# GlaireDaggers/Pretty-Fast-Video

Measured on AMD Instinct MI355X. Metric: macroblocks/s (encode+decode) 1080p YUV420, higher is better.
Workload: dtype i32 (encoder transforms evaluated in exact f32; decoders i32)

## Files before the change

pretty-fast-video_amd/csrc/pfv_kernels.hip:

```cpp
#include <hip/hip_runtime.h>
#include <stdint.h>

#include "pfv_device.h"
#include "pfv_prof.h"


namespace pfv {

namespace {
__constant__ int kScale[64] = {
    32, 37, 34, 26, 32, 26, 34, 37, 37, 43, 39, 31, 37, 31, 39, 43, 34, 39, 35, 28, 34, 28, 35, 39, 26, 31, 28, 22, 26, 22,
    28, 31, 32, 37, 34, 26, 32, 26, 34, 37, 26, 31, 28, 22, 26, 22, 28, 31, 34, 39, 35, 28, 34, 28, 35, 39, 37, 43, 39, 31,
    37, 31, 39, 43,
};
__constant__ int kInvZigzag[64] = {
    0,  1,  5,  6,  14, 15, 27, 28, 2,  4,  7,  13, 16, 26, 29, 42, 3,  8,  12, 17, 25, 30, 41, 43, 9,  11, 18, 24, 31, 40,
    44, 53, 10, 19, 23, 32, 39, 45, 52, 54, 20, 22, 33, 38, 46, 51, 55, 60, 21, 34, 37, 47, 50, 56, 59, 61, 35, 36, 48, 49,
    57, 58, 62, 63,
};
}

constexpr int kWinRows = 16 * kStripsPerWG + 30;
constexpr int kWinStride = 176;
constexpr int kWinBytes = kWinRows * kWinStride;
// ... 512 lines not shown
{
    return quant_div(quant_scale(m, scale16), rcp, magic, biased);
}
__device__ __forceinline__ f2 residual_f(f2 src, f2 pred)
{
    const f2 d = src - pred;
    const float c = 0.5f - 1.0f / 2048.0f;
    const f2 r = f2{__builtin_fmaf(d[0], c, kQuantMagic), __builtin_fmaf(d[1], c, kQuantMagic)};
    return f2{__builtin_fmaf(r[0], 256.0f, -256.0f * kQuantMagic), __builtin_fmaf(r[1], 256.0f, -256.0f * kQuantMagic)};
}
__device__ __forceinline__ int16_t quant_low16(float biased) { return (int16_t)__float_as_int(biased); }
__device__ __forceinline__ void forward_half_f(f2 (&x)[8], int *xw, int m, int i, const LaneQ &lq, float magic)
{
    int *mb = xw + m * kMBPitch;
    ffdct8(x);
    f_rows_to_cols(x, mb, i, m & 3);
    ffdct8(x);
    int16_t *stage = reinterpret_cast<int16_t *>(xw) + m * (2 * kStagePitch);
#pragma unroll
    for (int k = 0; k < 8; k++) {
        const int zz = lq.zz(k);
        f2 biased;
        x[k] = quant_pair_f(x[k], lq.scale(k), lq.rcp(k), magic, biased);
#pragma unroll
        for (int s = 0; s < 2; s++) stage[s * 64 + zz] = quant_low16(biased[s]);
    }
    wave_lds_sync();
}
constexpr float kPixelBias = 127.501953125f;
__device__ __forceinline__ f2 iframe_pixel_f(f2 x) { return x * f2s(1.0f / 256.0f) + f2s(kPixelBias); }
template <bool PIXEL>
__device__ __forceinline__ void inverse_half_f(f2 (&c)[8], int *xw, int m, int i, const LaneQ &lq)
{
    int *mb = xw + m * kMBPitch;
#pragma unroll
    for (int k = 0; k < 8; k++) c[k] = c[k] * f2s(lq.deqf(k));
    fidct8(c);
    f_cols_to_rows(c, mb, i, m & 3);
    fidct8(c);
#pragma unroll
    for (int k = 0; k < 8; k++) c[k] = PIXEL ? iframe_pixel_f(c[k]) : f2floor(c[k] * f2s(1.0f / 256.0f));
}
__device__ __forceinline__ uint4 pack_row_f(const f2 (&px)[8])
{
    unsigned w[4] = {0, 0, 0, 0};
#pragma unroll
    for (int k = 0; k < 8; k++) {
        w[k >> 2] = __builtin_amdgcn_cvt_pk_u8_f32(px[k][0], (unsigned)(k & 3), w[k >> 2]);
        w[2 + (k >> 2)] = __builtin_amdgcn_cvt_pk_u8_f32(px[k][1], (unsigned)(k & 3), w[2 + (k >> 2)]);
    }
    return make_uint4(w[0], w[1], w[2], w[3]);
}
__device__ __forceinline__ void unpack_row_f(const uint4 &row, f2 (&px)[8])
{
#pragma unroll
    for (int k = 0; k < 4; k++) {
        px[k] = f2{(float)byte_of(row.x, k), (float)byte_of(row.z, k)};
        px[k + 4] = f2{(float)byte_of(row.y, k), (float)byte_of(row.w, k)};
    }
}

template <bool FLT, int LPM = 8>
__global__ __launch_bounds__(kThreads) void k_enc_iframe(FrameGeom g, const uint8_t *__restrict__ src,
                                                          int16_t *__restrict__ coef, uint8_t *__restrict__ recon,
                                                          const QTab *__restrict__ qtabs, float qmagic)
{
    __shared__ __attribute__((aligned(16))) int xchg[kStripsPerWG][kXchgDwords];
    __shared__ __attribute__((aligned(16))) int qtab_lds[kStripsPerWG][kQTabDwords];
    constexpr int kPasses = LPM == 8 ? 2 : 1;

    const int lane = threadIdx.x & 63, wave = __builtin_amdgcn_readfirstlane((int)(threadIdx.x >> 6));
    const int gw = xcd_remap((int)blockIdx.x, (int)gridDim.x) * kStripsPerWG + wave;
    const int gstrip = LPM == 8 ? gw : gw >> 1, half_strip = LPM == 8 ? 0 : gw & 1;
    if (gstrip >= g.strips_per_frame * g.n_streams) return;
    const StripPos sp = locate_strip(g, gstrip);
    if (half_strip * 4 >= sp.n_mb) return;
    const PlaneGeom &p = g.p[sp.plane];
    const int slot = lane >> 3, i = lane & 7;
    const int m = LPM == 8 ? slot : half_strip * 4 + (slot >> 1);
    int *xw = xchg[wave];

    fill_qtable<true, FLT>(qtab_lds[wave], qtabs + p.qsel, lane);
    const uint8_t *plane = frame_src(g, src, sp.stream) + p.src_off;
    uint4 rows[kPasses];
#pragma unroll
    for (int pass = 0; pass < kPasses; pass++) rows[pass] = load_src16(plane, p, sp.x0 + m * 16, sp.y0 + i + 8 * (LPM == 8 ? pass : (slot & 1)));

    wave_lds_sync();
    const LaneQ lq{qtab_lds[wave], i};
    int16_t *coef_mb0 = coef + ((long)sp.stream * g.mbs_per_frame + sp.mb_first) * 256;
    uint8_t *dst = recon ? recon + (long)sp.stream * g.pad_frame_bytes + p.pad_off + (long)(sp.y0 + i) * p.pw + sp.x0 + m * 16
                         : nullptr;
#pragma unroll
    for (int pass = 0; pass < kPasses; pass++) {
        const int h = LPM == 8 ? pass : (slot & 1);
        if (FLT) {
            f2 x[8];
            unpack_row_f(rows[pass], x);
#pragma unroll
            for (int k = 0; k < 8; k++) x[k] = x[k] * f2s(256.0f) - f2s(32768.0f);
            forward_half_f(x, xw, slot, i, lq, qmagic);
            if (LPM == 8) store_coef_half(xw, coef_mb0, sp.n_mb, lane, h);
            else store_coef_quads(xw, coef_mb0, sp.n_mb, lane, half_strip);
            wave_lds_sync();
            if (recon) {
                inverse_half_f<true>(x, xw, slot, i, lq);
                if (m < sp.n_mb) *reinterpret_cast<uint4 *>(dst + (long)(8 * h) * p.pw) = pack_row_f(x);
            }
        } else {
            int v[2][8];
            unpack_row(rows[pass], v);
#pragma unroll
            for (int s = 0; s < 2; s++) {
#pragma unroll
                for (int k = 0; k < 8; k++) v[s][k] = (int)((unsigned)(v[s][k] - 128) << 8);
            }
            forward_half(v, xw, slot, i, lq, true);
            if (LPM == 8) store_coef_half(xw, coef_mb0, sp.n_mb, lane, h);
            else store_coef_quads(xw, coef_mb0, sp.n_mb, lane, half_strip);
            wave_lds_sync();
            if (recon) {
                inverse_half(v, xw, slot, i, lq);
#pragma unroll
                for (int s = 0; s < 2; s++)
#pragma unroll
                    for (int k = 0; k < 8; k++) v[s][k] = min(max(v[s][k] + 128, 0), 255);
                if (m < sp.n_mb) *reinterpret_cast<uint4 *>(dst + (long)(8 * h) * p.pw) = pack_row(v);
            }
        }
    }
}

struct SearchState {
    int cx, cy;
    int err;
};

__device__ __forceinline__ unsigned dot_ab(const uint4 &a, unsigned b0, unsigned b1, unsigned b2, unsigned b3, unsigned acc)
{
    acc = __builtin_amdgcn_udot4(a.x, b0, acc, false);
    acc = __builtin_amdgcn_udot4(a.y, b1, acc, false);
    acc = __builtin_amdgcn_udot4(a.z, b2, acc, false);
    return __builtin_amdgcn_udot4(a.w, b3, acc, false);
}
__device__ __forceinline__ unsigned sq2(unsigned x, unsigned y, unsigned acc)
{
    return __builtin_amdgcn_udot4(y, y, __builtin_amdgcn_udot4(x, x, acc, false), false);
}
__device__ __forceinline__ unsigned sq4(unsigned b0, unsigned b1, unsigned b2, unsigned b3, unsigned acc) { return sq2(b2, b3, sq2(b0, b1, acc)); }

constexpr int kPencSplit = -1;
constexpr int kPsWaves = 7;
constexpr int kTfWaves = 7;
constexpr int kPencCompactMax = 16;
constexpr int kRedPitch = 72;
constexpr int kRedDwords = kStripMB * kRedPitch;
struct SearchLane {
    int neg2;
    int ord;
    int dy, dx;
    int *wr;
    const int4 *rd;
};
__device__ __forceinline__ SearchLane make_search_lane(int *red, int m, int i, int neg2)
{
    SearchLane sl;
    sl.neg2 = neg2;
    sl.ord = i + 1;
    const int b9 = i < 4 ? i : i + 1;
    sl.dy = b9 / 3 - 1;
    sl.dx = b9 - (b9 / 3) * 3 - 1;
    sl.wr = red + m * kRedPitch + i;
    sl.rd = reinterpret_cast<const int4 *>(red + m * kRedPitch + i * 8);
    return sl;
}
__device__ __forceinline__ unsigned mb_min(unsigned v)
{
    v = min(v, (unsigned)dpp<kQuadXor1>((int)v));
    v = min(v, (unsigned)dpp<kQuadXor2>((int)v));
    v = min(v, (unsigned)dpp<kRowHalfMirror>((int)v));
    return v;
}

template <int S, bool FIRST, bool BOUNDS, bool DPPRED = false>
__device__ __forceinline__ void search_level(const uint8_t *win, int wrow0, int wcol0, const uint4 &top, const uint4 &bot,
                                             int a2, int mbx, int mby, int pw, int ph, SearchState &st, const SearchLane &sl)
{
    constexpr bool kAligned = (S >= 4);
    const int sh = (st.cx - 1) & 3;
    const int col = kAligned ? (wcol0 + st.cx - S) : (S == 2 ? wcol0 + st.cx - 4 : wcol0 + ((st.cx - 1) & ~3));
    int part[3][3];
    if (S == 8) {
        unsigned ab[3][3] = {{0, 0, 0}, {0, 0, 0}, {0, 0, 0}}, bb[3][3] = {{0, 0, 0}, {0, 0, 0}, {0, 0, 0}};
#pragma unroll
        for (int j = 0; j < 4; j++) {
            const uint8_t *rp = win + (wrow0 + st.cy + (j - 1) * 8) * kWinStride + col;
            const uint2 p0 = *reinterpret_cast<const uint2 *>(rp), p2 = *reinterpret_cast<const uint2 *>(rp + 24);
            const uint4 p1 = *reinterpret_cast<const uint4 *>(rp + 8);
            const unsigned d[8] = {p0.x, p0.y, p1.x, p1.y, p1.z, p1.w, p2.x, p2.y};
            const unsigned q23 = sq2(d[2], d[3], 0), q45 = sq2(d[4], d[5], 0);
            const unsigned rsq[3] = {sq2(d[0], d[1], q23), q23 + q45, sq2(d[6], d[7], q45)};
#pragma unroll
            for (int c = 0; c < 3; c++) {
                if (j <= 2) {
                    ab[j][c] = dot_ab(top, d[2 * c], d[2 * c + 1], d[2 * c + 2], d[2 * c + 3], ab[j][c]);
                    bb[j][c] += rsq[c];
                }
                if (j >= 1) {
                    ab[j - 1][c] = dot_ab(bot, d[2 * c], d[2 * c + 1], d[2 * c + 2], d[2 * c + 3], ab[j - 1][c]);
                    bb[j - 1][c] += rsq[c];
                }
            }
        }
#pragma unroll
        for (int my = 0; my < 3; my++)
#pragma unroll
            for (int c = 0; c < 3; c++) part[my][c] = __mul24((int)ab[my][c], sl.neg2) + (int)bb[my][c];
    } else
#pragma unroll
    for (int my = -1; my <= 1; my++) {
        const uint8_t *rp = win + (wrow0 + st.cy + my * S) * kWinStride + col;
        const bool centre_known = !FIRST && my == 0;
        unsigned ab[3] = {0, 0, 0}, bb[3] = {0, 0, 0};
        if (S == 4) {
            const unsigned *t = reinterpret_cast<const unsigned *>(rp), *b = reinterpret_cast<const unsigned *>(rp + 8 * kWinStride);
            uint4 t1, b1;
            {
                const uint2 ta = *reinterpret_cast<const uint2 *>(rp + 4), tb = *reinterpret_cast<const uint2 *>(rp + 12);
                const uint2 ba = *reinterpret_cast<const uint2 *>(rp + 8 * kWinStride + 4), bc = *reinterpret_cast<const uint2 *>(rp + 8 * kWinStride + 12);
                t1 = make_uint4(ta.x, ta.y, tb.x, tb.y);
                b1 = make_uint4(ba.x, ba.y, bc.x, bc.y);
            }
            const unsigned dT[6] = {t[0], t1.x, t1.y, t1.z, t1.w, t[5]};
            const unsigned dB[6] = {b[0], b1.x, b1.y, b1.z, b1.w, b[5]};
#pragma unroll
            for (int c = 0; c < 3; c++) {
                if (centre_known && c == 1) continue;
                ab[c] = dot_ab(bot, dB[c], dB[c + 1], dB[c + 2], dB[c + 3], dot_ab(top, dT[c], dT[c + 1], dT[c + 2], dT[c + 3], 0));
            }
            const unsigned q23 = sq2(dB[2], dB[3], sq2(dT[2], dT[3], 0));
            if (centre_known) {
                bb[0] = sq2(dB[0], dB[1], sq2(dT[0], dT[1], q23));
                bb[2] = sq2(dB[4], dB[5], sq2(dT[4], dT[5], q23));
            } else {
                const unsigned y = __builtin_amdgcn_udot4(dB[1], dB[1], __builtin_amdgcn_udot4(dT[1], dT[1], q23, false), false);
                const unsigned z = __builtin_amdgcn_udot4(dB[4], dB[4], __builtin_amdgcn_udot4(dT[4], dT[4], 0, false), false);
                bb[0] = __builtin_amdgcn_udot4(dB[0], dB[0], __builtin_amdgcn_udot4(dT[0], dT[0], y, false), false);
                bb[1] = y + z;
                bb[2] = __builtin_amdgcn_udot4(dB[5], dB[5], __builtin_amdgcn_udot4(dT[5], dT[5], q23 + z, false), false);
            }
        } else if (S == 2) {
            const unsigned *t = reinterpret_cast<const unsigned *>(rp), *b = reinterpret_cast<const unsigned *>(rp + 8 * kWinStride);
            unsigned rt[6], rb[6];
#pragma unroll
            for (int k = 0; k < 6; k++) { rt[k] = t[k]; rb[k] = b[k]; }
#pragma unroll
            for (int c = 0; c < 3; c++) {
                if (centre_known && c == 1) continue;
                unsigned eT[4], eB[4];
#pragma unroll
                for (int k = 0; k < 4; k++) {
                    const int o = k + (c >> 1);
                    eT[k] = c == 1 ? rt[k + 1] : __builtin_amdgcn_alignbyte(rt[o + 1], rt[o], 2);
                    eB[k] = c == 1 ? rb[k + 1] : __builtin_amdgcn_alignbyte(rb[o + 1], rb[o], 2);
                }
                ab[c] = dot_ab(bot, eB[0], eB[1], eB[2], eB[3], dot_ab(top, eT[0], eT[1], eT[2], eT[3], 0));
#ifdef PFV_ABL_SEARCH_BB
                if (my != 0) continue;
#endif
                bb[c] = sq4(eB[0], eB[1], eB[2], eB[3], sq4(eT[0], eT[1], eT[2], eT[3], 0));
            }
        } else {
            const unsigned *t = reinterpret_cast<const unsigned *>(rp), *b = reinterpret_cast<const unsigned *>(rp + 8 * kWinStride);
            static_assert(S == 1 || S == 2 || S >= 4, "the byte-granular path is the 1-pixel level");
            unsigned rt[6], rb[6], dT[5], dB[5];
#pragma unroll
            for (int k = 0; k < 6; k++) { rt[k] = t[k]; rb[k] = b[k]; }
#pragma unroll
            for (int k = 0; k < 5; k++) {
                dT[k] = __builtin_amdgcn_alignbyte(rt[k + 1], rt[k], sh);
                dB[k] = __builtin_amdgcn_alignbyte(rb[k + 1], rb[k], sh);
            }
#pragma unroll
            for (int c = 0; c < 3; c++) {
                if (centre_known && c == 1) continue;
                unsigned eT[4], eB[4];
#pragma unroll
                for (int k = 0; k < 4; k++) {
                    eT[k] = c ? __builtin_amdgcn_alignbyte(dT[k + 1], dT[k], c) : dT[k];
                    eB[k] = c ? __builtin_amdgcn_alignbyte(dB[k + 1], dB[k], c) : dB[k];
                }
                ab[c] = dot_ab(bot, eB[0], eB[1], eB[2], eB[3], dot_ab(top, eT[0], eT[1], eT[2], eT[3], 0));
#ifdef PFV_ABL_SEARCH_BB
                if (my != 0) continue;
#endif
                bb[c] = sq4(eB[0], eB[1], eB[2], eB[3], sq4(eT[0], eT[1], eT[2], eT[3], 0));
            }
        }
#pragma unroll
        for (int c = 0; c < 3; c++) part[my + 1][c] = __mul24((int)ab[c], sl.neg2) + (int)bb[c];
    }
    int err;
    if (DPPRED) {
        const int v[8] = {part[0][0], part[0][1], part[0][2], part[1][0], part[1][2], part[2][0], part[2][1], part[2][2]};
        const int i = sl.ord - 1;
        const bool b2 = (i & 4) != 0, b1 = (i & 2) != 0, b0 = (i & 1) != 0;
        int k4[4], k2[2];
#pragma unroll
        for (int k = 0; k < 4; k++) k4[k] = (b2 ? v[4 + k] : v[k]) + dpp<kRowHalfMirror>(b2 ? v[k] : v[4 + k]);
#pragma unroll
        for (int k = 0; k < 2; k++) k2[k] = (b1 ? k4[2 + k] : k4[k]) + dpp<kQuadXor2>(b1 ? k4[k] : k4[2 + k]);
        err = a2 + (b0 ? k2[1] : k2[0]) + dpp<kQuadXor1>(b0 ? k2[0] : k2[1]);
    } else {
    int ord = 0;
#pragma unroll
    for (int my = -1; my <= 1; my++) {
#pragma unroll
        for (int mx = -1; mx <= 1; mx++) {
            if (my == 0 && mx == 0) continue;
            sl.wr[ord * 8] = part[my + 1][mx + 1];
            ord++;
        }
    }
    wave_lds_sync();
    const int4 x = sl.rd[0], y = sl.rd[1];
    wave_lds_sync();
    err = a2 + ((x.x + x.y) + (x.z + x.w)) + ((y.x + y.y) + (y.z + y.w));
    }
    bool valid = true;
    if (BOUNDS) {
        const int oy = mby + st.cy + sl.dy * S, ox = mbx + st.cx + sl.dx * S;
        valid = oy >= 0 && oy <= ph - 16 && ox >= 0 && ox <= pw - 16;
    }
    const unsigned key = valid ? (((unsigned)err << 4) | (unsigned)sl.ord) : 0xffffffffu;
    const unsigned centre = FIRST ? ((unsigned)(a2 + mb_sum(part[1][1])) << 4) : ((unsigned)st.err << 4);
    const unsigned best = min(mb_min(key), centre);
    const int bo = (int)(best & 15u);
    st.err = (int)(best >> 4);
    st.cy += ((int)((0x2A501u >> (2 * bo)) & 3u) - 1) * S;
    st.cx += ((int)((0x24891u >> (2 * bo)) & 3u) - 1) * S;
}

#ifndef PFV_PENC_WAVES
#define PFV_PENC_WAVES 5
#endif
struct TilePos {
    StripPos sp;
    int plane_ty;
    int winx0, winy0;
    bool wave_valid;
};
__device__ __forceinline__ TilePos locate_tile(const FrameGeom &g, int vt, int wave)
{
    TilePos t;
    t.sp.stream = vt / g.tiles_per_frame;
    int tl = vt - t.sp.stream * g.tiles_per_frame;
    t.sp.plane = plane_of(g, tl, true);
    const PlaneGeom &p = g.p[t.sp.plane];
    tl -= p.tile0;
    t.plane_ty = tl / p.strips_x;
    t.sp.sx = tl - t.plane_ty * p.strips_x;
    t.sp.by = t.plane_ty * kStripsPerWG + wave;
    finish_strip(g, t.sp);
    t.wave_valid = t.sp.by < p.bh;
    t.winx0 = t.sp.x0 - 16;
    t.winy0 = t.plane_ty * (16 * kStripsPerWG) - 15;
    return t;
}

__device__ __forceinline__ void issue_window(const PlaneGeom &p, const uint8_t *refp, const TilePos &t, uint8_t *winbuf, int wave,
                                             int lane)
{
    const int q0 = win_first_issue(wave), q1 = win_first_issue(wave + 1);
#pragma unroll 5
    for (int q = q0; q < q1; q++) {
        const int c = q * 64 + lane;
        const int row = c / kWinChunksPerRow, col = c - row * kWinChunksPerRow;
        const int y = min(max(t.winy0 + row, 0), p.ph - 1), x = min(max(t.winx0 + col * 16, 0), p.pw - 16);
        __builtin_amdgcn_global_load_lds((gbl_cvoid_t *)(refp + (long)y * p.pw + x), (lds_void_t *)(winbuf + c * 16), 16, 0, 0);
    }
}

struct SearchOut {
    int cx, cy;
    int err;
    bool coded;
    uint4 patch[2];
};

template <bool DPPRED = false>
__device__ __forceinline__ void penc_search(const FrameGeom &g, const TilePos &tp, const uint8_t *win, int *red, const uint4 (&rows)[2], int lane,
                                            float min_err, int neg2, SearchOut &so)
{
    const StripPos &sp = tp.sp;
    const PlaneGeom &p = g.p[sp.plane];
    const int m = lane >> 3, i = lane & 7;
    const bool mb_valid = m < sp.n_mb;
    const int mbx = sp.x0 + m * 16, mby = sp.y0;
    const int wcol0 = mbx - tp.winx0;
    const int wrow0 = mby - tp.winy0 + i;

    unsigned s2 = 0;
#pragma unroll
    for (int h = 0; h < 2; h++) {
        s2 = __builtin_amdgcn_udot4(rows[h].x, rows[h].x, s2, false);
        s2 = __builtin_amdgcn_udot4(rows[h].y, rows[h].y, s2, false);
        s2 = __builtin_amdgcn_udot4(rows[h].z, rows[h].z, s2, false);
        s2 = __builtin_amdgcn_udot4(rows[h].w, rows[h].w, s2, false);
    }
    const int a2 = mb_sum((int)s2);

    SearchState st;
    st.cx = 0; st.cy = 0; st.err = 0;
    const SearchLane sl = make_search_lane(red, m, i, neg2);
    const bool interior = sp.x0 >= 16 && sp.x0 + kStripMB * 16 + 16 <= p.pw && sp.y0 >= 16 && sp.y0 + 32 <= p.ph;
    if (interior) {
        search_level<8, true, false, DPPRED>(win, wrow0, wcol0, rows[0], rows[1], a2, mbx, mby, p.pw, p.ph, st, sl);
        KMARK(3);
        search_level<4, false, false, DPPRED>(win, wrow0, wcol0, rows[0], rows[1], a2, mbx, mby, p.pw, p.ph, st, sl);
        KMARK(4);
        search_level<2, false, false, DPPRED>(win, wrow0, wcol0, rows[0], rows[1], a2, mbx, mby, p.pw, p.ph, st, sl);
        KMARK(5);
        search_level<1, false, false, DPPRED>(win, wrow0, wcol0, rows[0], rows[1], a2, mbx, mby, p.pw, p.ph, st, sl);
        KMARK(6);
    } else {
        search_level<8, true, true, DPPRED>(win, wrow0, wcol0, rows[0], rows[1], a2, mbx, mby, p.pw, p.ph, st, sl);
        search_level<4, false, true, DPPRED>(win, wrow0, wcol0, rows[0], rows[1], a2, mbx, mby, p.pw, p.ph, st, sl);
        search_level<2, false, true, DPPRED>(win, wrow0, wcol0, rows[0], rows[1], a2, mbx, mby, p.pw, p.ph, st, sl);
        search_level<1, false, true, DPPRED>(win, wrow0, wcol0, rows[0], rows[1], a2, mbx, mby, p.pw, p.ph, st, sl);
    }

    so.coded = mb_valid && !((float)st.err <= min_err);
    so.cx = st.cx; so.cy = st.cy;
    so.err = st.err;

    const int wx = wcol0 + st.cx, shp = wx & 3;
    const uint8_t *rp = win + (wrow0 + st.cy) * kWinStride + (wx & ~3);
#pragma unroll
    for (int h = 0; h < 2; h++) {
        const unsigned *d = reinterpret_cast<const unsigned *>(rp + 8 * h * kWinStride);
        unsigned d0 = d[0], d1 = d[1], d2 = d[2], d3 = d[3], d4 = d[4];
        so.patch[h] = make_uint4(__builtin_amdgcn_alignbyte(d1, d0, shp), __builtin_amdgcn_alignbyte(d2, d1, shp),
                                 __builtin_amdgcn_alignbyte(d3, d2, shp), __builtin_amdgcn_alignbyte(d4, d3, shp));
    }
}

__device__ __forceinline__ void opaque_row(uint4 &r)
{
#ifndef PFV_HIPEMU
    asm volatile("" : "+v"(r.x), "+v"(r.y), "+v"(r.z), "+v"(r.w));
#else
    (void)r;
#endif
}
template <bool FLT, bool REUNPACK = false, class Store>
__device__ __forceinline__ uint4 penc_half(const uint4 &srow, const uint4 &prow, int *xw, int m, int i, const LaneQ &lq, float qmagic, bool want_recon,
                                           Store &&store)
{
    uint4 out = prow;
    if (FLT) {
        f2 x[8], pp[8];
        unpack_row_f(srow, x);
        unpack_row_f(prow, pp);
#pragma unroll
        for (int k = 0; k < 8; k++) x[k] = residual_f(x[k], pp[k]);
        forward_half_f(x, xw, m, i, lq, qmagic);
        store();
        wave_lds_sync();
        if (want_recon) {
            inverse_half_f<false>(x, xw, m, i, lq);
            if (REUNPACK) {
                uint4 again = prow;
                opaque_row(again);
                unpack_row_f(again, pp);
            }
#pragma unroll
            for (int k = 0; k < 8; k++) {
                const f2 t = f2{__builtin_fminf(x[k][0], 127.0f), __builtin_fminf(x[k][1], 127.0f)};
                pp[k] = pp[k] + t * f2s(2.0f);
            }
            out = pack_row_f(pp);
        }
    } else {
        int v[2][8], pp[2][8];
        unpack_row(srow, v);
        unpack_row(prow, pp);
#pragma unroll
        for (int s = 0; s < 2; s++) {
#pragma unroll
            for (int k = 0; k < 8; k++) {
                int d = v[s][k] - pp[s][k];
                v[s][k] = (int)((unsigned)tdiv2(d) << 8);
            }
        }
        forward_half(v, xw, m, i, lq, true);
        store();
        wave_lds_sync();
        if (want_recon) {
            inverse_half(v, xw, m, i, lq);
#pragma unroll
            for (int s = 0; s < 2; s++) {
#pragma unroll
                for (int k = 0; k < 8; k++)
                    pp[s][k] = min(max(pp[s][k] + 2 * v[s][k], 0), 255);
            }
            out = pack_row(pp);
        }
    }
    return out;
}

__device__ __forceinline__ void penc_store_skipped(int16_t *coef_mb, uint8_t *dst, long pw, int i, const uint4 (&patch)[2])
{
#pragma unroll
    for (int j = 0; j < 4; j++) st_stream(&reinterpret_cast<uint4 *>(coef_mb)[j * 8 + i], make_uint4(0, 0, 0, 0));
    if (dst) {
        *reinterpret_cast<uint4 *>(dst) = patch[0];
        *reinterpret_cast<uint4 *>(dst + 8 * pw) = patch[1];
    }
}

template <bool FLT>
__device__ __forceinline__ void penc_transform(const FrameGeom &g, const TilePos &tp, const SearchOut &so, const uint4 (&rows)[2], int *xw,
                                               int lane, int16_t *__restrict__ coef, uint8_t *__restrict__ recon, const int *qtab_lds, float qmagic)
{
    const StripPos &sp = tp.sp;
    const PlaneGeom &p = g.p[sp.plane];
    const int m = lane >> 3, i = lane & 7;
    const bool mb_valid = m < sp.n_mb, coded = so.coded;
    const int mbx = sp.x0 + m * 16;
    int16_t *coef_mb0 = coef + ((long)sp.stream * g.mbs_per_frame + sp.mb_first) * 256;
    uint8_t *dst = recon ? recon + (long)sp.stream * g.pad_frame_bytes + p.pad_off + (long)(sp.y0 + i) * p.pw + mbx : nullptr;

    if (__any(coded)) {
        const LaneQ lq{qtab_lds, i};
#pragma unroll
        for (int h = 0; h < 2; h++) {
            const uint4 o = penc_half<FLT>(coded ? rows[h] : so.patch[h], so.patch[h], xw, m, i, lq, qmagic, recon != nullptr,
                                           [&]() { store_coef_half(xw, coef_mb0, sp.n_mb, lane, h); });
            if (h == 0) KMARK(9);
            if (recon && mb_valid) *reinterpret_cast<uint4 *>(dst + (long)(8 * h) * p.pw) = o;
        }
    } else if (mb_valid) {
        penc_store_skipped(coef_mb0 + m * 256, dst, p.pw, i, so.patch);
    }
}

template <bool FLT>
__device__ __forceinline__ void penc_transform_compact(const FrameGeom &g, const TilePos &tp, int wave, int n_coded, const int *slot_orig,
                                                       const uint4 *staged, int *xw, int lane, int16_t *__restrict__ coef,
                                                       uint8_t *__restrict__ recon, const int *qtab_lds, float qmagic)
{
    const PlaneGeom &p = g.p[tp.sp.plane];
    const int m = lane >> 3, i = lane & 7;
    const int slot = wave * 8 + m;
    const bool has = slot < n_coded;
    const long tile_mb0 = (long)tp.sp.stream * g.mbs_per_frame + p.mb0 + (long)(tp.plane_ty * kStripsPerWG) * p.bw + tp.sp.sx * kStripMB;
    const LaneQ lq{qtab_lds, i};
    const uint4 *sl = staged + (has ? slot : 0) * 32 + i * 4;
#pragma unroll
    for (int h = 0; h < 2; h++) {
        uint4 srow = sl[h], prow = sl[2 + h];
        if (!has) srow = prow = make_uint4(0, 0, 0, 0);
        const uint4 o = penc_half<FLT>(srow, prow, xw, m, i, lq, qmagic, recon != nullptr, [&]() {
#pragma unroll
            for (int j = 0; j < 2; j++) {
                const int ch = j * 64 + lane, sc = wave * 8 + (ch >> 4);
                if (sc < n_coded) {
                    const int og = slot_orig[sc];
                    int16_t *mb = coef + (tile_mb0 + (long)(og >> 3) * p.bw + (og & 7)) * 256;
                    st_stream(&reinterpret_cast<uint4 *>(mb)[h * 16 + (ch & 15)], reinterpret_cast<const uint4 *>(xw)[stage_chunk(ch)]);
                }
            }
        });
        if (recon && has) {
            const int orig = slot_orig[slot];
            uint8_t *dst = recon + (long)tp.sp.stream * g.pad_frame_bytes + p.pad_off +
                           (long)((tp.plane_ty * kStripsPerWG + (orig >> 3)) * 16 + i + 8 * h) * p.pw + tp.sp.x0 + (orig & 7) * 16;
            *reinterpret_cast<uint4 *>(dst) = o;
        }
    }
}

template <bool FLT>
__global__ __launch_bounds__(kThreads) PFV_WAVES_PER_EU(PFV_PENC_WAVES) void k_enc_pframe(FrameGeom g, const uint8_t *__restrict__ src,
                                                          const uint8_t *__restrict__ ref, int8_t *__restrict__ mv_out,
                                                          uint8_t *__restrict__ has_out, int16_t *__restrict__ coef,
                                                          uint8_t *__restrict__ recon, const QTab *__restrict__ qtabs,
                                                          float min_err, int neg2, float qmagic, int compact_max)
{
    __shared__ __attribute__((aligned(16))) uint8_t win_lds[16 + kWinAlloc];
    __shared__ __attribute__((aligned(16))) int red_lds[kStripsPerWG][kRedDwords];
    __shared__ __attribute__((aligned(16))) int qtab_lds[kQTabDwords];
    uint8_t *win = win_lds + 16;

    const int lane = threadIdx.x & 63, wave = __builtin_amdgcn_readfirstlane((int)(threadIdx.x >> 6));
    const int m = lane >> 3, i = lane & 7;
    const int vt = xcd_remap((int)blockIdx.x, (int)gridDim.x);
    const TilePos cur = locate_tile(g, vt, wave);
    const PlaneGeom &p = g.p[cur.sp.plane];
    if (wave == 0) fill_qtable<true, FLT>(qtab_lds, qtabs + p.qsel, lane);

    KMARK(0);
    KMARK_WHERE();
    issue_window(p, ref + (long)cur.sp.stream * g.pad_frame_bytes + p.pad_off, cur, win, wave, lane);
    uint4 rows[2];
    rows[0] = rows[1] = make_uint4(0, 0, 0, 0);
    if (cur.wave_valid) {
        const uint8_t *plane = frame_src(g, src, cur.sp.stream) + p.src_off;
        rows[0] = load_src16(plane, p, cur.sp.x0 + m * 16, cur.sp.y0 + i);
        rows[1] = load_src16(plane, p, cur.sp.x0 + m * 16, cur.sp.y0 + i + 8);
    }
    KMARK(1);
    __syncthreads();
    KMARK(2);
    SearchOut so;
    so.cx = so.cy = 0; so.coded = false;
    so.patch[0] = so.patch[1] = make_uint4(0, 0, 0, 0);
    if (cur.wave_valid) penc_search(g, cur, win, red_lds[wave], rows, lane, min_err, neg2, so);
    KMARK(7);
    const bool mb_valid = cur.wave_valid && m < cur.sp.n_mb;
    if (i == 0 && mb_valid) {
        const long mbi = (long)cur.sp.stream * g.mbs_per_frame + cur.sp.mb_first + m;
        mv_out[mbi * 2 + 0] = (int8_t)so.cx;
        mv_out[mbi * 2 + 1] = (int8_t)so.cy;
        has_out[mbi] = so.coded ? 1 : 0;
    }
    constexpr int kMaskAt = (kStripsPerWG - 1) * kRedDwords + kRedDwords - 8;
    int *red_all = &red_lds[0][0];
    {
        const unsigned long long bal = __ballot(so.coded);
        unsigned mine = 0;
#pragma unroll
        for (int k = 0; k < kStripMB; k++) mine |= (unsigned)((bal >> (8 * k)) & 1ull) << k;
        if (lane == 0) red_all[kMaskAt + wave] = (int)mine;
    }
    __syncthreads();
    KMARK(8);
    unsigned tile_mask = 0;
#pragma unroll
    for (int k = 0; k < kStripsPerWG; k++) tile_mask |= (unsigned)__builtin_amdgcn_readfirstlane(red_all[kMaskAt + k]) << (8 * k);
    int n_coded = __builtin_popcount(tile_mask), strips_coded = 0;
#pragma unroll
    for (int k = 0; k < kStripsPerWG; k++) strips_coded += ((tile_mask >> (8 * k)) & 0xffu) ? 1 : 0;
    int *xw = reinterpret_cast<int *>(win + win_first_issue(wave) * 1024);
    constexpr int kCompactMax = kPencCompactMax;
    constexpr int kSlotOrigAt = kCompactMax * 128;
    static_assert(kSlotOrigAt + kCompactMax <= kMaskAt, "staging area + slot table must fit below the strip masks");
    static_assert(kStripsPerWG * 8 <= 32, "one bit per macroblock of the tile");
    if (n_coded <= compact_max && ((n_coded + 7) >> 3) < strips_coded) {
        uint4 *stage4 = reinterpret_cast<uint4 *>(red_all);
        const int place = wave * 8 + m;
        if (so.coded) {
            const int slot = __builtin_popcount(tile_mask & ((1u << place) - 1u));
            uint4 *sl = stage4 + slot * 32 + i * 4;
            sl[0] = rows[0]; sl[1] = rows[1]; sl[2] = so.patch[0]; sl[3] = so.patch[1];
            if (i == 0) red_all[kSlotOrigAt + slot] = place;
        } else if (mb_valid) {
            const PlaneGeom &pp = g.p[cur.sp.plane];
            penc_store_skipped(coef + ((long)cur.sp.stream * g.mbs_per_frame + cur.sp.mb_first + m) * 256,
                               recon ? recon + (long)cur.sp.stream * g.pad_frame_bytes + pp.pad_off + (long)(cur.sp.y0 + i) * pp.pw + cur.sp.x0 + m * 16 : nullptr,
                               pp.pw, i, so.patch);
        }
        __syncthreads();
        if (wave * 8 < n_coded)
            penc_transform_compact<FLT>(g, cur, wave, n_coded, red_all + kSlotOrigAt, stage4, xw, lane, coef, recon, qtab_lds, qmagic);
    } else if (cur.wave_valid) {
        penc_transform<FLT>(g, cur, so, rows, xw, lane, coef, recon, qtab_lds, qmagic);
    }
    KMARK(11);
}

template <bool DPPRED>
__global__ __launch_bounds__(kThreads) PFV_WAVES_PER_EU(kPsWaves) void k_pf_search(FrameGeom g, const uint8_t *__restrict__ src,
                                                          const uint8_t *__restrict__ ref, int8_t *__restrict__ mv_out,
                                                          uint8_t *__restrict__ has_out, int16_t *__restrict__ coef,
                                                          uint8_t *__restrict__ recon, float min_err, int neg2)
{
    __shared__ __attribute__((aligned(16))) uint8_t win_lds[16 + kWinAlloc];
    __shared__ __attribute__((aligned(16))) int red_lds[DPPRED ? 1 : kStripsPerWG][DPPRED ? 4 : kRedDwords];
    uint8_t *win = win_lds + 16;

    const int lane = threadIdx.x & 63, wave = __builtin_amdgcn_readfirstlane((int)(threadIdx.x >> 6));
    const int m = lane >> 3, i = lane & 7;
    const int vt = xcd_remap((int)blockIdx.x, (int)gridDim.x);
    const TilePos cur = locate_tile(g, vt, wave);
    const PlaneGeom &p = g.p[cur.sp.plane];
    issue_window(p, ref + (long)cur.sp.stream * g.pad_frame_bytes + p.pad_off, cur, win, wave, lane);
    uint4 rows[2];
    rows[0] = rows[1] = make_uint4(0, 0, 0, 0);
    if (cur.wave_valid) {
        const uint8_t *plane = frame_src(g, src, cur.sp.stream) + p.src_off;
        rows[0] = load_src16(plane, p, cur.sp.x0 + m * 16, cur.sp.y0 + i);
        rows[1] = load_src16(plane, p, cur.sp.x0 + m * 16, cur.sp.y0 + i + 8);
    }
    __syncthreads();
    if (!cur.wave_valid) return;
    SearchOut so;
    penc_search<DPPRED>(g, cur, win, red_lds[DPPRED ? 0 : wave], rows, lane, min_err, neg2, so);
    if (m < cur.sp.n_mb) {
        const long mbi = (long)cur.sp.stream * g.mbs_per_frame + cur.sp.mb_first + m;
        if (i == 0) {
            mv_out[mbi * 2 + 0] = (int8_t)so.cx;
            mv_out[mbi * 2 + 1] = (int8_t)so.cy;
            has_out[mbi] = so.coded ? 1 : 0;
        }
        if (!so.coded)
            penc_store_skipped(coef + mbi * 256, recon ? recon + (long)cur.sp.stream * g.pad_frame_bytes + p.pad_off + (long)(cur.sp.y0 + i) * p.pw + cur.sp.x0 + m * 16 : nullptr,
                               p.pw, i, so.patch);
    }
}

constexpr int kTfStrips = 8;
__host__ __device__ __forceinline__ int tf_groups_of_plane(const PlaneGeom &p) { return (p.strips_x * p.bh + kTfStrips - 1) / kTfStrips; }
__host__ __device__ __forceinline__ int tf_groups_per_frame(const FrameGeom &g)
{
    int n = 0;
    for (int k = 0; k < g.n_planes; k++) n += tf_groups_of_plane(g.p[k]);
    return n;
}

template <bool FLT>
__global__ __launch_bounds__(64) PFV_WAVES_PER_EU(kTfWaves) void k_pf_transform(FrameGeom g, const uint8_t *__restrict__ src, const uint8_t *__restrict__ ref,
                                                     const int8_t *__restrict__ mv, const uint8_t *__restrict__ has, int16_t *__restrict__ coef,
                                                     uint8_t *__restrict__ recon, const QTab *__restrict__ qtabs, float qmagic)
{
    __shared__ __attribute__((aligned(16))) int xw[kXchgDwords];
    __shared__ __attribute__((aligned(16))) int qtab_lds[kQTabDwords];
    __shared__ __attribute__((aligned(16))) int strip_tab[kTfStrips][4];
    __shared__ int slot_tab[64];
    __shared__ int pass_mbi[kStripMB];

    const int lane = threadIdx.x & 63, m = lane >> 3, i = lane & 7;
    const int gpf = tf_groups_per_frame(g);
    const int gq = xcd_remap((int)blockIdx.x, (int)gridDim.x);
    const int stream = gq / gpf;
    int gr = gq - stream * gpf, plane = 0;
    for (; plane + 1 < g.n_planes && gr >= tf_groups_of_plane(g.p[plane]); plane++) gr -= tf_groups_of_plane(g.p[plane]);
    const PlaneGeom &p = g.p[plane];
    const int strips_p = p.strips_x * p.bh;
    const int s_first = gr * kTfStrips;

    bool coded = false;
    int cxy = 0;
    {
        const int s = s_first + m;
        const int by = s / p.strips_x, sx = s - by * p.strips_x;
        const int n_mb = min(kStripMB, p.bw - sx * kStripMB), mb_first = p.mb0 + by * p.bw + sx * kStripMB;
        if (i == 0) reinterpret_cast<int4 *>(strip_tab[m])[0] = make_int4(sx * (kStripMB * 16), by * 16, mb_first, 0);
        if (s < strips_p && i < n_mb) {
            const long mbi = (long)stream * g.mbs_per_frame + mb_first + i;
            if (has[mbi]) {
                coded = true;
                cxy = ((int)mv[mbi * 2 + 0] & 0xff) << 8 | ((int)mv[mbi * 2 + 1] & 0xff) << 16;
            }
        }
    }
    const unsigned long long bal = __ballot(coded);
    const int n_coded = __builtin_popcountll(bal);
    if (n_coded == 0) return;
    if (coded) slot_tab[__builtin_amdgcn_mbcnt_hi((unsigned)(bal >> 32), __builtin_amdgcn_mbcnt_lo((unsigned)bal, 0u))] = lane | cxy;
    fill_qtable<true, FLT>(qtab_lds, qtabs + p.qsel, lane);
    wave_lds_sync();

    const LaneQ lq{qtab_lds, i};
    const uint8_t *splane = frame_src(g, src, stream) + p.src_off;
    const uint8_t *rplane = ref + (long)stream * g.pad_frame_bytes + p.pad_off;
    uint8_t *oplane = recon ? recon + (long)stream * g.pad_frame_bytes + p.pad_off : nullptr;
    int16_t *coef_frame = coef + (long)stream * g.mbs_per_frame * 256;
    for (int k0 = 0; k0 < n_coded; k0 += kStripMB) {
        const bool has_slot = k0 + m < n_coded;
        if (i == 0) {
            int mbf = -1;
            if (has_slot) {
                const int e = slot_tab[k0 + m];
                mbf = strip_tab[(e >> 3) & 7][2] + (e & 7);
            }
            pass_mbi[m] = mbf;
        }
#pragma unroll
        for (int h = 0; h < 2; h++) {
            uint4 srow = make_uint4(0, 0, 0, 0), prow = srow;
            if (has_slot) {
                const int e = slot_tab[k0 + m];
                const int4 st = reinterpret_cast<const int4 *>(strip_tab[(e >> 3) & 7])[0];
                const int mbx = st.x + (e & 7) * 16, y = st.y + i + 8 * h;
                const int cx = (int)(int8_t)(e >> 8), cy = (int)(int8_t)(e >> 16);
                srow = load_src16(splane, p, mbx, y);
                prow = load_unaligned16(rplane + (long)(y + cy) * p.pw + (mbx + cx));
            }
            const uint4 o = penc_half<FLT, true>(srow, prow, xw, m, i, lq, qmagic, recon != nullptr, [&]() {
#pragma unroll
                for (int j = 0; j < 2; j++) {
                    const int ch = j * 64 + lane, mbf = pass_mbi[ch >> 4];
                    if (mbf >= 0)
                        st_stream(&reinterpret_cast<uint4 *>(coef_frame + (long)mbf * 256)[h * 16 + (ch & 15)], reinterpret_cast<const uint4 *>(xw)[stage_chunk(ch)]);
                }
            });
            if (oplane && has_slot) {
                const int e = slot_tab[k0 + m];
                const int4 st = reinterpret_cast<const int4 *>(strip_tab[(e >> 3) & 7])[0];
                *reinterpret_cast<uint4 *>(oplane + (long)(st.y + i + 8 * h) * p.pw + st.x + (e & 7) * 16) = o;
            }
        }
        wave_lds_sync();
    }
}

constexpr int kThreads16 = 64 * 2 * kStripsPerWG;
constexpr int kWaves16 = 2 * kStripsPerWG;
constexpr int kRedPitch16 = 144;
static_assert(4 * kRedPitch16 <= kRedDwords, "the 16-lane reduction layout fits the reduction region");
static_assert(kStripsPerWG * kXchgDwords * 4 <= kWinAlloc && kStripsPerWG * kXchgDwords <= kWaves16 * kRedDwords, "exchange regions of 8 wavefronts");
__device__ __forceinline__ constexpr int win_first_issue16(int w) { return (w * kWinIssues + kWaves16 - 1) / kWaves16; }
constexpr int kRowRor8 = 0x128;

__device__ __forceinline__ int mb_sum16(int v)
{
    v = mb_sum(v);
// ... 503 lines not shown
```

Measured before the change: 1.422 billion.

## Compact P-frame transforms at half-macroblock granularity with a unified LDS layout

New measurement: 1.434 billion, median of 6. Within noise of the previous version (+0.9%).

```diff
diff --git a/pretty-fast-video_amd/csrc/pfv_kernels.hip b/pretty-fast-video_amd/csrc/pfv_kernels.hip
--- a/pretty-fast-video_amd/csrc/pfv_kernels.hip
+++ b/pretty-fast-video_amd/csrc/pfv_kernels.hip
@@ -688,7 +688,7 @@
 constexpr int kPencSplit = -1;
 constexpr int kPsWaves = 7;
 constexpr int kTfWaves = 7;
-constexpr int kPencCompactMax = 16;
+constexpr int kPencCompactMax = 28;
 constexpr int kRedPitch = 72;
 constexpr int kRedDwords = kStripMB * kRedPitch;
 struct SearchLane {
@@ -989,6 +989,13 @@
     (void)r;
 #endif
 }
+__device__ __forceinline__ int opaque_lane(int l)
+{
+#ifndef PFV_HIPEMU
+    asm volatile("" : "+v"(l));
+#endif
+    return l;
+}
 template <bool FLT, bool REUNPACK = false, class Store>
 __device__ __forceinline__ uint4 penc_half(const uint4 &srow, const uint4 &prow, int *xw, int m, int i, const LaneQ &lq, float qmagic, bool want_recon,
                                            Store &&store)
@@ -1083,41 +1090,62 @@
 }
 
 template <bool FLT>
-__device__ __forceinline__ void penc_transform_compact(const FrameGeom &g, const TilePos &tp, int wave, int n_coded, const int *slot_orig,
+__device__ __forceinline__ void penc_transform_compact(const FrameGeom &g, const TilePos &tp, int wave, int n_coded, const int *rank_place,
                                                        const uint4 *staged, int *xw, int lane, int16_t *__restrict__ coef,
                                                        uint8_t *__restrict__ recon, const int *qtab_lds, float qmagic)
 {
     const PlaneGeom &p = g.p[tp.sp.plane];
     const int m = lane >> 3, i = lane & 7;
-    const int slot = wave * 8 + m;
-    const bool has = slot < n_coded;
     const long tile_mb0 = (long)tp.sp.stream * g.mbs_per_frame + p.mb0 + (long)(tp.plane_ty * kStripsPerWG) * p.bw + tp.sp.sx * kStripMB;
     const LaneQ lq{qtab_lds, i};
-    const uint4 *sl = staged + (has ? slot : 0) * 32 + i * 4;
-#pragma unroll
-    for (int h = 0; h < 2; h++) {
-        uint4 srow = sl[h], prow = sl[2 + h];
-        if (!has) srow = prow = make_uint4(0, 0, 0, 0);
+    static_assert(kPencCompactMax <= 2 * kStripsPerWG * 4, "two passes per wavefront take every staged macroblock");
+#pragma unroll
+    for (int k = 0; k < 2; k++) {
+        const int r0 = (k * kStripsPerWG + wave) * 4;
+        if (r0 >= n_coded) break;
+        uint4 srow, prow;
+        {
+            const int l = opaque_lane(lane), rank = r0 + (l >> 4);
+            const bool has = rank < n_coded;
+            const uint4 *sl = staged + (has ? rank : 0) * 32 + (l & 7) * 4 + ((l >> 3) & 1);
+            srow = sl[0]; prow = sl[2];
+            if (!has) srow = prow = make_uint4(0, 0, 0, 0);
+        }
         const uint4 o = penc_half<FLT>(srow, prow, xw, m, i, lq, qmagic, recon != nullptr, [&]() {
+            const int l = opaque_lane(lane);
 #pragma unroll
             for (int j = 0; j < 2; j++) {
-                const int ch = j * 64 + lane, sc = wave * 8 + (ch >> 4);
-                if (sc < n_coded) {
-                    const int og = slot_orig[sc];
+                const int ch = j * 64 + l, rc = r0 + (ch >> 5);
+                if (rc < n_coded) {
+                    const int og = rank_place[rc];
                     int16_t *mb = coef + (tile_mb0 + (long)(og >> 3) * p.bw + (og & 7)) * 256;
-                    st_stream(&reinterpret_cast<uint4 *>(mb)[h * 16 + (ch & 15)], reinterpret_cast<const uint4 *>(xw)[stage_chunk(ch)]);
+                    st_stream(&reinterpret_cast<uint4 *>(mb)[ch & 31], reinterpret_cast<const uint4 *>(xw)[stage_chunk(ch)]);
                 }
             }
         });
-        if (recon && has) {
-            const int orig = slot_orig[slot];
+        const int l = opaque_lane(lane), rank = r0 + (l >> 4);
+        if (recon && rank < n_coded) {
+            const int orig = rank_place[rank];
             uint8_t *dst = recon + (long)tp.sp.stream * g.pad_frame_bytes + p.pad_off +
-                           (long)((tp.plane_ty * kStripsPerWG + (orig >> 3)) * 16 + i + 8 * h) * p.pw + tp.sp.x0 + (orig & 7) * 16;
+                           (long)((tp.plane_ty * kStripsPerWG + (orig >> 3)) * 16 + (l & 15)) * p.pw + tp.sp.x0 + (orig & 7) * 16;
             *reinterpret_cast<uint4 *>(dst) = o;
         }
     }
 }
 
+constexpr int kPencWinAt = 16;
+constexpr int kPencRedAt = kPencWinAt + kWinAlloc;
+constexpr int kPencStageAt = kPencWinAt + kStripsPerWG * kXchgDwords * 4;
+constexpr int kPencTailAt = kPencRedAt + kStripsPerWG * kRedDwords * 4;
+constexpr int kPencRankAt = kPencStageAt + kPencCompactMax * 512;
+constexpr int kPencMaskAt = kPencRankAt + 32 * 4;
+constexpr int kPencQTabAt = kPencMaskAt + kStripsPerWG * 4;
+constexpr int kPencLdsBytes = kPencQTabAt + kQTabDwords * 4;
+static_assert(kPencStageAt <= kPencRedAt && kPencStageAt % 16 == 0, "the staging area starts behind the last exchange region, inside the window");
+static_assert(kPencRankAt >= kPencTailAt && kPencCompactMax <= 32, "the staging area covers the reduction regions; one table entry per staged macroblock");
+static_assert(kPencRedAt % 16 == 0 && kPencQTabAt % 16 == 0, "16-byte accesses to the reduction regions and the quantiser tables");
+static_assert((kPencLdsBytes + 1279) / 1280 * 1280 * (PFV_PENC_WAVES * 4 / kStripsPerWG) <= 160 * 1024,
+              "LDS of PFV_PENC_WAVES wavefronts per SIMD, rounded up to a 1280-byte allocation granule");
 template <bool FLT>
 __global__ __launch_bounds__(kThreads) PFV_WAVES_PER_EU(PFV_PENC_WAVES) void k_enc_pframe(FrameGeom g, const uint8_t *__restrict__ src,
                                                           const uint8_t *__restrict__ ref, int8_t *__restrict__ mv_out,
@@ -1125,10 +1153,9 @@
                                                           uint8_t *__restrict__ recon, const QTab *__restrict__ qtabs,
                                                           float min_err, int neg2, float qmagic, int compact_max)
 {
-    __shared__ __attribute__((aligned(16))) uint8_t win_lds[16 + kWinAlloc];
-    __shared__ __attribute__((aligned(16))) int red_lds[kStripsPerWG][kRedDwords];
-    __shared__ __attribute__((aligned(16))) int qtab_lds[kQTabDwords];
-    uint8_t *win = win_lds + 16;
+    __shared__ __attribute__((aligned(16))) uint8_t lds[kPencLdsBytes];
+    uint8_t *win = lds + kPencWinAt;
+    int *qtab_lds = reinterpret_cast<int *>(lds + kPencQTabAt);
 
     const int lane = threadIdx.x & 63, wave = __builtin_amdgcn_readfirstlane((int)(threadIdx.x >> 6));
     const int m = lane >> 3, i = lane & 7;
@@ -1153,7 +1180,7 @@
     SearchOut so;
     so.cx = so.cy = 0; so.coded = false;
     so.patch[0] = so.patch[1] = make_uint4(0, 0, 0, 0);
-    if (cur.wave_valid) penc_search(g, cur, win, red_lds[wave], rows, lane, min_err, neg2, so);
+    if (cur.wave_valid) penc_search(g, cur, win, reinterpret_cast<int *>(lds + kPencRedAt) + wave * kRedDwords, rows, lane, min_err, neg2, so);
     KMARK(7);
     const bool mb_valid = cur.wave_valid && m < cur.sp.n_mb;
     if (i == 0 && mb_valid) {
@@ -1162,36 +1189,34 @@
         mv_out[mbi * 2 + 1] = (int8_t)so.cy;
         has_out[mbi] = so.coded ? 1 : 0;
     }
-    constexpr int kMaskAt = (kStripsPerWG - 1) * kRedDwords + kRedDwords - 8;
-    int *red_all = &red_lds[0][0];
+    int *masks = reinterpret_cast<int *>(lds + kPencMaskAt);
     {
         const unsigned long long bal = __ballot(so.coded);
         unsigned mine = 0;
 #pragma unroll
         for (int k = 0; k < kStripMB; k++) mine |= (unsigned)((bal >> (8 * k)) & 1ull) << k;
-        if (lane == 0) red_all[kMaskAt + wave] = (int)mine;
+        if (lane == 0) masks[wave] = (int)mine;
     }
     __syncthreads();
     KMARK(8);
     unsigned tile_mask = 0;
 #pragma unroll
-    for (int k = 0; k < kStripsPerWG; k++) tile_mask |= (unsigned)__builtin_amdgcn_readfirstlane(red_all[kMaskAt + k]) << (8 * k);
+    for (int k = 0; k < kStripsPerWG; k++) tile_mask |= (unsigned)__builtin_amdgcn_readfirstlane(masks[k]) << (8 * k);
     int n_coded = __builtin_popcount(tile_mask), strips_coded = 0;
 #pragma unroll
     for (int k = 0; k < kStripsPerWG; k++) strips_coded += ((tile_mask >> (8 * k)) & 0xffu) ? 1 : 0;
-    int *xw = reinterpret_cast<int *>(win + win_first_issue(wave) * 1024);
-    constexpr int kCompactMax = kPencCompactMax;
-    constexpr int kSlotOrigAt = kCompactMax * 128;
-    static_assert(kSlotOrigAt + kCompactMax <= kMaskAt, "staging area + slot table must fit below the strip masks");
+    int *xw = reinterpret_cast<int *>(win) + wave * kXchgDwords;
     static_assert(kStripsPerWG * 8 <= 32, "one bit per macroblock of the tile");
-    if (n_coded <= compact_max && ((n_coded + 7) >> 3) < strips_coded) {
-        uint4 *stage4 = reinterpret_cast<uint4 *>(red_all);
+    static_assert((kPencCompactMax + 1 + 3) / 4 >= 2 * kStripsPerWG, "no tile with more than kPencCompactMax coded macroblocks saves a pass");
+    if (n_coded <= compact_max && ((n_coded + 3) >> 2) < 2 * strips_coded) {
+        uint4 *stage4 = reinterpret_cast<uint4 *>(lds + kPencStageAt);
+        int *rank_place = reinterpret_cast<int *>(lds + kPencRankAt);
         const int place = wave * 8 + m;
         if (so.coded) {
-            const int slot = __builtin_popcount(tile_mask & ((1u << place) - 1u));
-            uint4 *sl = stage4 + slot * 32 + i * 4;
+            const int rank = __builtin_popcount(tile_mask & ((1u << place) - 1u));
+            uint4 *sl = stage4 + rank * 32 + i * 4;
             sl[0] = rows[0]; sl[1] = rows[1]; sl[2] = so.patch[0]; sl[3] = so.patch[1];
-            if (i == 0) red_all[kSlotOrigAt + slot] = place;
+            if (i == 0) rank_place[rank] = place;
         } else if (mb_valid) {
             const PlaneGeom &pp = g.p[cur.sp.plane];
             penc_store_skipped(coef + ((long)cur.sp.stream * g.mbs_per_frame + cur.sp.mb_first + m) * 256,
@@ -1199,8 +1224,7 @@
                                pp.pw, i, so.patch);
         }
         __syncthreads();
-        if (wave * 8 < n_coded)
-            penc_transform_compact<FLT>(g, cur, wave, n_coded, red_all + kSlotOrigAt, stage4, xw, lane, coef, recon, qtab_lds, qmagic);
+        penc_transform_compact<FLT>(g, cur, wave, n_coded, rank_place, stage4, xw, lane, coef, recon, qtab_lds, qmagic);
     } else if (cur.wave_valid) {
         penc_transform<FLT>(g, cur, so, rows, xw, lane, coef, recon, qtab_lds, qmagic);
     }
```
